# nihui/rife-ncnn-vulkan

Measured on AMD Instinct MI355X. Metric: interpolated frames/sec (rife-v4.6, 3840x2160), higher is better.
Workload: dtype f16x2-split MFMA + f32 accumulate (fp32-equivalent; activations stored f32 or as {hi, lo} f16 pairs); 1 GPU; rife-v4.6 3840x2160 frame pairs resident in HBM, timestep sweep [0.5, 0.125, 0.25, 0.7, 0.9], synthetic seeded weights; pairs_in_flight_per_gpu=4, cu_partition=every stream owns 1 / 2 of the compute units (rife_hip_stream_create), frames=F1: images/0.png, 1.png of the reference tiled 6 x 6, parallelism=frame pairs sharded over ranks, no data-path collective

## Files before the change

### rife-ncnn-vulkan_amd/__init__.py

```python
import ctypes
import os

import numpy as np

_HERE = os.path.dirname(os.path.abspath(__file__))
LIB_PATH = os.environ.get("RIFE_HIP_LIB") or os.path.join(_HERE, "librife_hip.so")
TEST_LIB_PATH = os.path.join(_HERE, "librife_hip_test.so")
_lib = None
_testlib = None

C_ABI_SYMBOLS = [
    "rife_hip_device_count", "rife_hip_create", "rife_hip_destroy", "rife_hip_load", "rife_hip_process",
    "rife_hip_process_device", "rife_hip_process_device_batch", "rife_hip_stream_create", "rife_hip_stream_destroy", "rife_hip_process_batch", "rife_hip_frame_upload", "rife_hip_process_frames", "rife_hip_frame_release",
    "rife_hip_last_error", "rife_hip_profile_enable", "rife_hip_profile_read",
    "rife_hip_host_alloc", "rife_hip_host_free", "rife_hip_host_register", "rife_hip_host_unregister",
    "rife_hip_graph_check", "rife_hip_param_hash",
    "rife_hip_frame_bytes", "rife_hip_process_px", "rife_hip_process_device_px", "rife_hip_process_device_batch_px", "rife_hip_frame_upload_px",
    "rife_hip_image_check", "rife_hip_image_row_bytes", "rife_hip_process_image", "rife_hip_process_device_image", "rife_hip_frame_upload_image", "rife_hip_process_frames_image",
]
PIX_RGB8, PIX_RGB10_U16, PIX_A2B10G10R10 = 0, 1, 2
PIX_RGBA8 = 4
PIX_NV12, PIX_I420, PIX_P010, PIX_I420P10 = 16, 17, 18, 19
PIX_I422, PIX_I422P10, PIX_I444, PIX_I444P10 = 33, 35, 49, 51
_YUV_FORMATS = (PIX_NV12, PIX_I420, PIX_P010, PIX_I420P10, PIX_I422, PIX_I422P10, PIX_I444, PIX_I444P10)
# ... 526 lines not shown
        _check(self._L.rife_hip_profile_enable(self._h, int(on)), "profile_enable", self._L)

    def profile_read(self):
        names = ctypes.create_string_buffer(4096)
        ms = np.zeros(64, np.float64); n = np.zeros(64, np.int64); fl = np.zeros(64, np.float64)
        k = self._L.rife_hip_profile_read(self._h, names, 4096, _p(ms), _p(n), _p(fl), 64)
        nm = names.value.decode().split("\n")
        return {nm[i]: dict(ms=float(ms[i]), launches=int(n[i]), flops=float(fl[i])) for i in range(k)}

    def _need_taps(self):
        if not self._taps:
            raise RifeError("the parity taps (include/rife_hip_test.h) live in the test build: create the engine with amd.test_build().RIFE(...)")

    def pool_state(self):
        self._need_taps()
        a, b, c = ctypes.c_int(), ctypes.c_int(), ctypes.c_int()
        _check(self._L.rife_hip_pool_state(self._h, ctypes.byref(a), ctypes.byref(b), ctypes.byref(c)), "pool_state", self._L)
        return a.value, b.value, c.value

    def v4_extract_flow(self, in0image, in1image, timestep, fi, inject=(), pixfmt=None):
        self._need_taps()
        px = _pix_of(in0image, pixfmt)
        if px is not None and _pix_of(in1image, px) != px:
            raise ValueError("both frames must have the same pixel format")
        if px is not None:
            a = np.ascontiguousarray(in0image); b = np.ascontiguousarray(in1image)
        else:
            a = np.ascontiguousarray(in0image, dtype=np.uint8); b = np.ascontiguousarray(in1image, dtype=np.uint8)
        h, w = a.shape[:2]
        nc, fh, fw = ctypes.c_int(), ctypes.c_int(), ctypes.c_int()
        _check(self._L.rife_hip_v4_flow_dims(self._h, w, h, fi, ctypes.byref(nc), ctypes.byref(fh), ctypes.byref(fw)), "v4_flow_dims", self._L)
        out = np.empty((nc.value, fh.value, fw.value), np.float32)
        inj = [np.ascontiguousarray(f, dtype=np.float32) for f in inject]
        arr = (ctypes.c_void_p * max(1, len(inj)))(*[f.ctypes.data for f in inj])
        if px is not None:
            _check(self._L.rife_hip_v4_extract_flow_px(self._h, _p(a), _p(b), w, h, float(timestep), fi, arr, len(inj), _p(out), px), "v4_extract_flow_px", self._L)
            return out
        _check(self._L.rife_hip_v4_extract_flow(self._h, _p(a), _p(b), w, h, float(timestep), fi, arr, len(inj), _p(out)), "v4_extract_flow", self._L)
        return out


    def v4_tap(self, in0image, in1image, timestep, what, b, inject, pixfmt=None):
        self._need_taps()
        px = _pix_of(in0image, pixfmt)
        if px is not None and _pix_of(in1image, px) != px:
            raise ValueError("both frames must have the same pixel format")
        if px is not None:
            a = np.ascontiguousarray(in0image); bb = np.ascontiguousarray(in1image)
        else:
            a = np.ascontiguousarray(in0image, dtype=np.uint8); bb = np.ascontiguousarray(in1image, dtype=np.uint8)
        h, w = a.shape[:2]
        wp, hp = (w + 31) // 32 * 32, (h + 31) // 32 * 32
        s = {1: 4, 2: 2, 3: 1}.get(b, 1)
        out = np.empty((4 if px == PIX_RGBA8 else 3, hp, wp) if what == 2 else (5, hp, wp) if what in (3, 4) else (12, hp // s, wp // s), np.float32)
        inj = [np.ascontiguousarray(f, dtype=np.float32) for f in inject]
        arr = (ctypes.c_void_p * max(1, len(inj)))(*[f.ctypes.data for f in inj])
        if px is not None:
            _check(self._L.rife_hip_v4_tap_px(self._h, _p(a), _p(bb), w, h, float(timestep), int(what), int(b), arr, len(inj), _p(out), px), "v4_tap_px", self._L)
            return out
        _check(self._L.rife_hip_v4_tap(self._h, _p(a), _p(bb), w, h, float(timestep), int(what), int(b), arr, len(inj), _p(out)), "v4_tap", self._L)
        return out

    def v4_process_injected(self, in0image, in1image, timestep, inject):
        self._need_taps()
        a = np.ascontiguousarray(in0image, dtype=np.uint8); bb = np.ascontiguousarray(in1image, dtype=np.uint8)
        h, w, _ = a.shape
        out = np.empty((h, w, 3), np.uint8)
        inj = [np.ascontiguousarray(f, dtype=np.float32) for f in inject]
        arr = (ctypes.c_void_p * max(1, len(inj)))(*[f.ctypes.data for f in inj])
        _check(self._L.rife_hip_v4_process_injected(self._h, _p(a), _p(bb), w, h, float(timestep), arr, len(inj), _p(out)), "v4_process_injected", self._L)
        return out


def op_conv3x3(x, weight, bias, stride=1, residual=None, slope=None, gpuid=0):
    x = np.ascontiguousarray(x, np.float32); weight = np.ascontiguousarray(weight, np.float32); bias = np.ascontiguousarray(bias, np.float32)
    c, h, w = x.shape
    oc = weight.shape[0]
    out = np.empty((oc, (h - 1) // stride + 1, (w - 1) // stride + 1), np.float32)
    res = None if residual is None else np.ascontiguousarray(residual, np.float32)
    sl = None if slope is None else np.ascontiguousarray(slope, np.float32)
    _check(testlib().rife_hip_op_conv3x3(gpuid, _p(x), c, h, w, _p(weight), _p(bias), oc, stride, _p(res), _p(sl), _p(out)), "op_conv3x3", testlib())
    return out


def op_deconv4x4(x, weight, bias, slope=None, gpuid=0):
    x = np.ascontiguousarray(x, np.float32); weight = np.ascontiguousarray(weight, np.float32); bias = np.ascontiguousarray(bias, np.float32)
    c, h, w = x.shape
    oc = weight.shape[0]
    out = np.empty((oc, 2 * h, 2 * w), np.float32)
    sl = None if slope is None else np.ascontiguousarray(slope, np.float32)
    _check(testlib().rife_hip_op_deconv4x4(gpuid, _p(x), c, h, w, _p(weight), _p(bias), oc, _p(sl), _p(out)), "op_deconv4x4", testlib())
    return out


def op_warp(image, flow, gpuid=0):
    image = np.ascontiguousarray(image, np.float32); flow = np.ascontiguousarray(flow, np.float32)
    c, h, w = image.shape
    out = np.empty_like(image)
    _check(testlib().rife_hip_op_warp(gpuid, _p(image), _p(flow), c, h, w, _p(out)), "op_warp", testlib())
    return out


def op_s16_geom(C, H, W):
    pitch, rows, plane, nbytes = ctypes.c_int(), ctypes.c_int(), ctypes.c_uint(), ctypes.c_size_t()
    _check(testlib().rife_hip_op_s16_geom(int(C), int(H), int(W), ctypes.byref(pitch), ctypes.byref(rows), ctypes.byref(plane), ctypes.byref(nbytes)), "op_s16_geom", testlib())
    return pitch.value, rows.value, plane.value, nbytes.value

# ... 50 lines not shown
```

### rife-ncnn-vulkan_amd/csrc/elementwise.h

```cpp
#pragma once
#include <hip/hip_runtime.h>
#include <stdint.h>

namespace rife {

__global__ void k_preproc(const uint8_t* __restrict__ rgb, int w, int h, uint32_t* __restrict__ out, int wp, int hp) {
    const int x = blockIdx.x * blockDim.x + threadIdx.x, y = blockIdx.y;
    if (x >= wp) return;
    uint32_t v = 0;
    if (x < w && y < h) {
        const uint8_t* p = rgb + ((size_t)y * w + x) * 3;
        v = (uint32_t)p[0] | ((uint32_t)p[1] << 8) | ((uint32_t)p[2] << 16);
    }
    out[(size_t)y * wp + x] = v;
}

__global__ void k_preproc4(const uint8_t* __restrict__ rgb, int w, int h, uint32_t* __restrict__ out, int wp, int hp) {
    const int x4 = (blockIdx.x * blockDim.x + threadIdx.x) * 4, y = blockIdx.y;
    if (x4 >= wp) return;
    uint4 v = make_uint4(0u, 0u, 0u, 0u);
    if (x4 < w && y < h) {
        typedef uint32_t u32x3 __attribute__((ext_vector_type(3)));
        u32x3 q;
        __builtin_memcpy(&q, __builtin_assume_aligned(rgb + ((size_t)y * w + x4) * 3, 4), 12);
// ... 150 lines not shown
    const int x = blockIdx.x * blockDim.x + threadIdx.x, y = blockIdx.y;
    if (x >= w) return;
    const size_t plane = (size_t)w * h;
    const WarpTaps t = warp_taps(x, y, flow[(size_t)y * w + x], flow[plane + (size_t)y * w + x], w, h);
    for (int q = 0; q < c; q++) {
        const float* im = image + q * plane;
        out[q * plane + (size_t)y * w + x] = warp_lerp(im[t.i00], im[t.i01], im[t.i10], im[t.i11], t.alpha, t.beta);
    }
}

__device__ __forceinline__ float down4(float v00, float v01, float v10, float v11) {
    const float r0 = v00 * 0.5f + v01 * 0.5f;
    const float r1 = v10 * 0.5f + v11 * 0.5f;
    return r0 * 0.5f + r1 * 0.5f;
}

template <int D>
__device__ __forceinline__ void assemble0_body(const uint32_t* __restrict__ img0, const uint32_t* __restrict__ img1, float timestep_arg, const float* __restrict__ tsp,
                                               float* __restrict__ X, int wp, int hp) {
    const float timestep = tsp ? *tsp : timestep_arg;
    const int Wb = wp / 8, Hb = hp / 8;
    const int x = blockIdx.x * blockDim.x + threadIdx.x, y = blockIdx.y;
    if (x >= Wb || y >= Hb) return;
    const int sx = 8 * x + 3, sy = 8 * y + 3;
    const size_t i00 = (size_t)sy * wp + sx, i10 = i00 + wp;
    const float3 a0 = unpack_rgb<D>(img0[i00]), a1 = unpack_rgb<D>(img0[i00 + 1]), a2 = unpack_rgb<D>(img0[i10]), a3 = unpack_rgb<D>(img0[i10 + 1]);
    const float3 b0 = unpack_rgb<D>(img1[i00]), b1 = unpack_rgb<D>(img1[i00 + 1]), b2 = unpack_rgb<D>(img1[i10]), b3 = unpack_rgb<D>(img1[i10 + 1]);
    float4 o0, o1;
    o0.x = down4(a0.x, a1.x, a2.x, a3.x); o0.y = down4(a0.y, a1.y, a2.y, a3.y); o0.z = down4(a0.z, a1.z, a2.z, a3.z);
    o0.w = down4(b0.x, b1.x, b2.x, b3.x); o1.x = down4(b0.y, b1.y, b2.y, b3.y); o1.y = down4(b0.z, b1.z, b2.z, b3.z);
    o1.z = down4(timestep, timestep, timestep, timestep);
    o1.w = 0.f;
    float4* dst = reinterpret_cast<float4*>(X + ((size_t)y * Wb + x) * 8);
    dst[0] = o0; dst[1] = o1;
}
__global__ void k_assemble0(const uint32_t* __restrict__ img0, const uint32_t* __restrict__ img1, float timestep_arg, const float* __restrict__ tsp,
                            float* __restrict__ X, int wp, int hp) {
    assemble0_body<8>(img0, img1, timestep_arg, tsp, X, wp, hp);
}
__global__ void k_assemble0_d10(const uint32_t* __restrict__ img0, const uint32_t* __restrict__ img1, float timestep_arg, const float* __restrict__ tsp,
                                float* __restrict__ X, int wp, int hp) {
    assemble0_body<10>(img0, img1, timestep_arg, tsp, X, wp, hp);
}

__device__ __forceinline__ void up_coeff(int d, int S, int in, int& s0, float& a0, float& a1) {
    float f = ((float)d + 0.5f) * (1.0f / (float)S) - 0.5f;
    int s = (int)floorf(f);
    f -= (float)s;
    if (s < 0) { s = 0; f = 0.f; }
    if (s >= in - 1) { s = in - 2; f = 1.f; }
    s0 = s; a0 = 1.f - f; a1 = f;
}

template <int S>
__device__ __forceinline__ void flow_upsampled(const float* __restrict__ flow, int wp, int hp, int x, int y, float4& u, float& um) {
    const int Wb = wp / S, Hb = hp / S;
    int sx, sy; float a0, a1, b0, b1;
    up_coeff(x, S, Wb, sx, a0, a1);
    up_coeff(y, S, Hb, sy, b0, b1);
    const float* p00 = flow + ((size_t)sy * Wb + sx) * 8;
    const float* p10 = p00 + (size_t)Wb * 8;
    const float4 q00 = *reinterpret_cast<const float4*>(p00), q01 = *reinterpret_cast<const float4*>(p00 + 8);
    const float4 q10 = *reinterpret_cast<const float4*>(p10), q11 = *reinterpret_cast<const float4*>(p10 + 8);
    const float m00 = p00[4], m01 = p00[12], m10 = p10[4], m11 = p10[12];
#define RIFE_UP(c00, c01, c10, c11) (((c00) * a0 + (c01) * a1) * b0 + ((c10) * a0 + (c11) * a1) * b1)
    u.x = RIFE_UP(q00.x, q01.x, q10.x, q11.x);
    u.y = RIFE_UP(q00.y, q01.y, q10.y, q11.y);
    u.z = RIFE_UP(q00.z, q01.z, q10.z, q11.z);
    u.w = RIFE_UP(q00.w, q01.w, q10.w, q11.w);
    um = RIFE_UP(m00, m01, m10, m11);
#undef RIFE_UP
}
template <int S>
__device__ __forceinline__ void flow_first(const float* __restrict__ flow, int wp, int hp, int x, int y, float4& f, float& m) {
    float4 u; float um;
    flow_upsampled<S>(flow, wp, hp, x, y, u, um);
    const float s = (float)S;
    f = make_float4(u.x * s, u.y * s, u.z * s, u.w * s);
    m = um;
}
template <int S>
__device__ __forceinline__ void flow_accumulate(const float4 u, const float um, float4& f, float& m) {
    const float s = (float)S;
    f = make_float4(f.x * 1.0f + u.x * s, f.y * 1.0f + u.y * s, f.z * 1.0f + u.z * s, f.w * 1.0f + u.w * s);
    m = m + um;
}

struct FlowPending {
    const float* flow = nullptr;
    float4* Fw = nullptr;
    float* Mw = nullptr;
};

template <int S, int UPD = 0, int D = 8>
__device__ __forceinline__ void assemble_pixel(const uint32_t* __restrict__ img0, const uint32_t* __restrict__ img1, float timestep,
                                               const float4* __restrict__ F, const float* __restrict__ M, int wp, int hp, int x, int y, float o[12],
                                               const FlowPending& pend = FlowPending{}) {
    if (S == 1) {
        const size_t i = (size_t)y * wp + x;
        float4 f; float mk;
        if (UPD == 2) flow_first<2 * S>(pend.flow, wp, hp, x, y, f, mk);
        else { f = F[i]; mk = M[i]; }
        if (UPD == 1) {
            float4 u; float um;
            flow_upsampled<2 * S>(pend.flow, wp, hp, x, y, u, um);
            flow_accumulate<2 * S>(u, um, f, mk);
            pend.Fw[i] = f; pend.Mw[i] = mk;
        }
        const float3 w0 = warp_rgbx<D>(img0, x, y, f.x, f.y, wp, hp);
        const float3 w1 = warp_rgbx<D>(img1, x, y, f.z, f.w, wp, hp);
        o[0] = w0.x; o[1] = w0.y; o[2] = w0.z; o[3] = w1.x; o[4] = w1.y; o[5] = w1.z; o[6] = timestep; o[7] = mk;
        o[8] = f.x; o[9] = f.y; o[10] = f.z; o[11] = f.w;
    } else {
        const int sx = S * x + S / 2 - 1, sy = S * y + S / 2 - 1;
        float v[4][12];
#pragma unroll
        for (int k = 0; k < 4; k++) {
            const int px = sx + (k & 1), py = sy + (k >> 1);
            const size_t i = (size_t)py * wp + px;
            float4 f; float mk;
            if (UPD == 2) flow_first<2 * S>(pend.flow, wp, hp, px, py, f, mk);
            else { f = F[i]; mk = M[i]; }
            if (UPD == 1) {
                float4 u; float um;
                flow_upsampled<2 * S>(pend.flow, wp, hp, px, py, u, um);
                flow_accumulate<2 * S>(u, um, f, mk);
                pend.Fw[i] = f; pend.Mw[i] = mk;
            }
            const float3 w0 = warp_rgbx<D>(img0, px, py, f.x, f.y, wp, hp);
            const float3 w1 = warp_rgbx<D>(img1, px, py, f.z, f.w, wp, hp);
            v[k][0] = w0.x; v[k][1] = w0.y; v[k][2] = w0.z; v[k][3] = w1.x; v[k][4] = w1.y; v[k][5] = w1.z;
            v[k][6] = timestep; v[k][7] = mk;
// ... 344 lines not shown
```

### rife-ncnn-vulkan_amd/csrc/engine.hip

```cpp
#include <hip/hip_runtime.h>

#include <algorithm>
#include <chrono>
#include <climits>
#include <cmath>
#include <cstdio>
#include <cstring>
#include <initializer_list>
#include <array>
#include <map>
#include <memory>
#include <atomic>
#include <mutex>
#include <string>
#include <thread>
#include <vector>

#if defined(RIFE_HIP_BENCH_BUILD) && !defined(RIFE_HIP_TEST_BUILD)
#define RIFE_HIP_TEST_BUILD 1
#endif
#include "../../include/rife_hip.h"
#ifdef RIFE_HIP_TEST_BUILD
#include "../../include/rife_hip_test.h"
#endif
#include "conv_mfma.h"
#include "conv_img.h"
#include "elementwise.h"
#include "yuv.h"
#include "planes.h"
#include "image_check.h"
#include "elementwise_v2.h"
#include "stem_fused.h"
#include "stem_fused_v2.h"
#include "stem_rs.h"
#include "tail_rs.h"
#include "head_h2.h"
#include "conv_t64.h"
#include "conv_row.h"
#include "conv_rs.h"
#include "conv_rs2.h"
#ifdef RIFE_HIP_TEST_BUILD
#include "conv_ks.h"
#endif
#include "graph_kernels.h"
#include "model_hashes.h"
#include "ncnn_model.h"

#include "engine_switches.h"
#include "engine_layers.h"
#include "engine_dispatch.h"
#include "engine_ctx.h"
#include "engine_v4.h"
#include "engine_v2.h"
#include "engine_v1.h"
#include "engine_abi.h"
#include "engine_image.h"
```

### rife-ncnn-vulkan_amd/csrc/engine_abi.h

```cpp

extern "C" {

const char* rife_hip_last_error(void) { return g_err.c_str(); }

int rife_hip_device_count(void) {
    int n = 0;
    if (hipGetDeviceCount(&n) != hipSuccess) return 0;
    return n;
}

rife_hip_t* rife_hip_create(int gpuid, int tta_mode, int tta_temporal_mode, int uhd_mode, int num_threads, int rife_v2, int rife_v4) {
    if (check_device(gpuid)) return nullptr;
    rife_hip* E = new rife_hip;
    E->gpuid = gpuid; E->tta = tta_mode; E->tta_temporal = tta_temporal_mode; E->uhd = uhd_mode;
    E->num_threads = num_threads; E->v2 = rife_v2; E->v4 = rife_v4;
    E->frame_pool = std::make_shared<FramePool>();
    E->frame_pool->gpuid = gpuid;
    const Switches sw = read_switches();
    E->t64 = sw.t64; E->rs = sw.rs; E->rs2 = sw.rs2; E->stem_rs = sw.stem_rs; E->tta_consensus = sw.tta_consensus;
    E->tail_rs = sw.tail_rs; E->tail_rs_always = sw.tail_rs_always; E->fuse_flow = sw.fuse_flow;
    if (sw.ks_mask >= 0) E->ks_mask = sw.ks_mask;
    if (E->fuse_flow) g_fuse_flow_buffers = true;
    return E;
}
// ... 768 lines not shown
    return n;
}

#ifdef RIFE_HIP_TEST_BUILD
static int rife_hip_v4_extract_flow_impl(const rife_hip_t* E, const uint8_t* in0, const uint8_t* in1, int w, int h, float timestep, int fi,
                                         const float* const* inject, int n_inject, float* out6chw, int pixfmt) {
    int rc;
    if ((rc = process_common(E, w, h, timestep))) return rc;
    if (!E->v4) return fail(RIFE_HIP_EINVAL, "stage taps exist for the rife-v4 family only");
    if (pix_bpp(pixfmt) == 0) return fail(RIFE_HIP_EINVAL, "unknown pixel format");
    if ((rc = pixfmt_supported(E, pixfmt))) return rc;
    if (fi < 0 || fi > 3 || n_inject < 0 || n_inject > fi) return fail(RIFE_HIP_EINVAL, "bad stage index");
    if ((rc = check_device(E->gpuid))) return rc;
    Ctx c;
    if (hipStreamCreateWithFlags(&c.stream, hipStreamNonBlocking) != hipSuccess) return fail(RIFE_HIP_EHIP, "hipStreamCreate failed");
    c.own_stream = true;
    if ((rc = ensure_ctx(c, w, h, pixfmt))) return rc;
    const size_t nbytes = frame_bytes(w, h, pixfmt);
    HIPCHK(hipMemcpyAsync(c.d_in0, in0, nbytes, hipMemcpyHostToDevice, c.stream));
    HIPCHK(hipMemcpyAsync(c.d_in1, in1, nbytes, hipMemcpyHostToDevice, c.stream));
    launch_preproc(c.stream, c.d_in0, c.w, c.h, c.img0, c.wp, c.hp, pixfmt);
    launch_preproc(c.stream, c.d_in1, c.w, c.h, c.img1, c.wp, c.hp, pixfmt);
    float* tmp = nullptr;
    if ((rc = dalloc(c, tmp, (size_t)c.wp * c.hp * 6))) return rc;
    const int nc = E->v40 ? 5 : 6;
    for (int b = 0; b <= fi; b++) {
        const int s = E->flow_div(b), Hb = c.hp / s, Wb = c.wp / s;
        if (b < n_inject) {
            HIPCHK(hipMemcpyAsync(tmp, inject[b], (size_t)Hb * Wb * nc * 4, hipMemcpyHostToDevice, c.stream));
            hipLaunchKernelGGL(k_chw_to_nhwc, grid2d(Wb, Hb), dim3(256), 0, c.stream, tmp, c.flow[b], nc, Hb, Wb, 8);
        } else {
            if ((rc = run_block_convs(*E, c, b, timestep))) return rc;
        }
        if (b < fi && (rc = run_flow_update(*E, c, b))) return rc;
    }
    const int s = E->flow_div(fi), Hb = c.hp / s, Wb = c.wp / s;
    hipLaunchKernelGGL(k_nhwc_to_chw, grid2d(Wb, Hb), dim3(256), 0, c.stream, c.flow[fi], tmp, nc, Hb, Wb, 8);
    HIPCHK(hipMemcpyAsync(out6chw, tmp, (size_t)Hb * Wb * nc * 4, hipMemcpyDeviceToHost, c.stream));
    HIPCHK(hipStreamSynchronize(c.stream));
    return 0;
}
int rife_hip_v4_extract_flow(const rife_hip_t* E, const uint8_t* in0, const uint8_t* in1, int w, int h, float timestep, int fi,
                             const float* const* inject, int n_inject, float* out6chw) {
    return rife_hip_v4_extract_flow_impl(E, in0, in1, w, h, timestep, fi, inject, n_inject, out6chw, RIFE_HIP_PIX_RGB8);
}
int rife_hip_v4_extract_flow_px(const rife_hip_t* E, const void* in0, const void* in1, int w, int h, float timestep, int fi, const float* const* inject,
                                int n_inject, float* out6chw, int pixfmt) {
    if (!in0 || !in1 || !out6chw) return fail(RIFE_HIP_EINVAL, "null frame / output pointer");
    try { return rife_hip_v4_extract_flow_impl(E, static_cast<const uint8_t*>(in0), static_cast<const uint8_t*>(in1), w, h, timestep, fi, inject, n_inject, out6chw, pixfmt); }
    catch (const std::exception& e) { return fail(RIFE_HIP_EINVAL, std::string("v4_extract_flow_px: ") + e.what()); }
}

static int tap_prologue(const rife_hip_t* E, Ctx& c, const uint8_t* in0, const uint8_t* in1, int w, int h, const float* const* inject, int n_inject, float*& tmp,
                        const float** pending = nullptr, int pixfmt = RIFE_HIP_PIX_RGB8) {
    int rc;
    if (hipStreamCreateWithFlags(&c.stream, hipStreamNonBlocking) != hipSuccess) return fail(RIFE_HIP_EHIP, "hipStreamCreate failed");
    c.own_stream = true;
    if ((rc = ensure_ctx(c, w, h, pixfmt))) return rc;
    const size_t nbytes = frame_bytes(w, h, pixfmt);
    HIPCHK(hipMemcpyAsync(c.d_in0, in0, nbytes, hipMemcpyHostToDevice, c.stream));
    HIPCHK(hipMemcpyAsync(c.d_in1, in1, nbytes, hipMemcpyHostToDevice, c.stream));
    launch_preproc(c.stream, c.d_in0, c.w, c.h, c.img0, c.wp, c.hp, pixfmt);
    launch_preproc(c.stream, c.d_in1, c.w, c.h, c.img1, c.wp, c.hp, pixfmt);
    if ((rc = dalloc(c, tmp, (size_t)c.wp * c.hp * 16))) return rc;
    for (int k = 0; k < n_inject; k++) {
        const int s = E->blk[k].scale, Hb = c.hp / s, Wb = c.wp / s;
        HIPCHK(hipMemcpyAsync(tmp, inject[k], (size_t)Hb * Wb * 6 * 4, hipMemcpyHostToDevice, c.stream));
        hipLaunchKernelGGL(k_chw_to_nhwc, grid2d(Wb, Hb), dim3(256), 0, c.stream, tmp, c.flow[k], 6, Hb, Wb, 8);
        if (pending && k == n_inject - 1 && k < 3 && flow_update_fused_into(*E, c, k + 1)) { *pending = c.flow[k]; continue; }
        if (k < 3 && (rc = run_flow_update(*E, c, k))) return rc;
    }
    HIPCHK(hipGetLastError());
    return 0;
}

static int rife_hip_v4_tap_impl(const rife_hip_t* E, const uint8_t* in0, const uint8_t* in1, int w, int h, float timestep, int what, int b,
                                const float* const* inject, int n_inject, float* out, int pixfmt = RIFE_HIP_PIX_RGB8) {
    int rc;
    if ((rc = process_common(E, w, h, timestep))) return rc;
    if (!E->v4 || E->v40) return fail(RIFE_HIP_EINVAL, "the gather taps exist for the rife-v4.6 graph only");
    if (pix_bpp(pixfmt) == 0) return fail(RIFE_HIP_EINVAL, "unknown pixel format");
    if ((rc = pixfmt_supported(E, pixfmt))) return rc;
    if (pixfmt && what == 3) return fail(RIFE_HIP_EINVAL, "tap 3 (an A/B form the product does not run) is served for RGB8 frames only");
    if (what < 0 || what > 5) return fail(RIFE_HIP_EINVAL, "bad tap");
    if (what == 5 && b != 3) return fail(RIFE_HIP_EINVAL, "the row-streaming stem kernel serves block 3");
    if (what == 2 ? n_inject != 4 : (b < 1 || b > 3 || n_inject != b)) return fail(RIFE_HIP_EINVAL, "bad block / injection count");
    if ((rc = check_device(E->gpuid))) return rc;
    Ctx c; float* tmp = nullptr;
    const float* pending = nullptr;
    if ((rc = tap_prologue(E, c, in0, in1, w, h, inject, n_inject, tmp, (what == 1 || what == 3) ? &pending : nullptr, pixfmt))) return rc;
    hipStream_t st = c.stream;
    auto copy_fm = [&](const float4* F, const float* M) -> int {
        hipLaunchKernelGGL(k_nhwc_to_chw, grid2d(c.wp, c.hp), dim3(256), 0, st, reinterpret_cast<const float*>(F), tmp, 4, c.hp, c.wp, 4);
        HIPCHK(hipGetLastError());
        const size_t P = (size_t)c.wp * c.hp;
        HIPCHK(hipMemcpyAsync(out, tmp, P * 16, hipMemcpyDeviceToHost, st));
        HIPCHK(hipMemcpyAsync(out + 4 * P, M, P * 4, hipMemcpyDeviceToHost, st));
        HIPCHK(hipStreamSynchronize(st));
        return 0;
    };
    if (what == 4) return copy_fm(c.F, c.M);
    if (what == 5) {
        const int Hq = c.hp / 4, Wq = c.wp / 4;
        const S16Geom G(Hq, Wq);
        const size_t nb = G.bytes(64), pl = G.plane();
        unsigned char* dout = nullptr; uint16_t *dw0 = nullptr, *dw1 = nullptr; float *dbias = nullptr, *dslope = nullptr;
        if ((rc = dalloc(c, dout, nb)) || (rc = dalloc(c, dw0, (size_t)9 * 2 * 32 * 8)) || (rc = dalloc(c, dw1, (size_t)2 * 9 * 2 * 64 * 8)) ||
            (rc = dalloc(c, dbias, 64)) || (rc = dalloc(c, dslope, 64))) return rc;
        std::vector<float> hz(64, 0.f), ho(64, 1.f);
        HIPCHK(hipMemcpyAsync(dbias, hz.data(), 256, hipMemcpyHostToDevice, st));
        HIPCHK(hipMemcpyAsync(dslope, ho.data(), 256, hipMemcpyHostToDevice, st));
        HIPCHK(hipFuncSetAttribute(reinterpret_cast<const void*>(stem_rs_kernel<0>), hipFuncAttributeMaxDynamicSharedMemorySize, SRS_LDS));
        HIPCHK(hipFuncSetAttribute(reinterpret_cast<const void*>(stem_rs_kernel<0, 10>), hipFuncAttributeMaxDynamicSharedMemorySize, SRS_LDS));
        std::vector<unsigned char> host(nb);
        int inv[32];
        for (int i = 0; i < 32; i++) inv[s16_row_channel(i)] = i;
        for (int g = 0; g < 2; g++)
            for (int ty = 1; ty <= 2; ty++)
                for (int tx = 1; tx <= 2; tx++) {
                    std::vector<uint16_t> h0((size_t)9 * 2 * 32 * 8, 0), h1((size_t)2 * 9 * 2 * 64 * 8, 0);
                    for (int j = 0; j < 2; j++)
                        for (int k = 0; k < 12; k++) h0[(((size_t)((1 + g) * 3 + 1 + j) * 2 + k / 8) * 32 + 12 * j + k) * 8 + k % 8] = f2h(1.f);
                    for (int oc = 0; oc < 24; oc++)
                        h1[((((size_t)(oc / 16) * 9 + ty * 3 + tx) * 2 + (oc % 16) / 8) * 64 + inv[oc]) * 8 + oc % 8] = f2h(1.f);
                    HIPCHK(hipMemcpyAsync(dw0, h0.data(), h0.size() * 2, hipMemcpyHostToDevice, st));
                    HIPCHK(hipMemcpyAsync(dw1, h1.data(), h1.size() * 2, hipMemcpyHostToDevice, st));
                    HIPCHK(hipMemsetAsync(dout, 0, nb, st));
                    StemRsArgs a;
                    a.img0 = c.img0; a.img1 = c.img1; a.F = c.F; a.M = c.M; a.w0 = dw0; a.bias0 = dbias; a.slope0 = dslope; a.w1 = dw1; a.bias1 = dbias; a.slope1 = dslope;
                    a.out = dout; a.timestep = timestep; a.tsp = nullptr; a.wp = c.wp; a.hp = c.hp; a.Hq = Hq; a.Wq = Wq; a.pitch = G.pitch; a.plane = G.plane();
                    a.nunits = ((Wq + SRS_SW - 1) / SRS_SW) * Hq;
                    const int nwg = std::min(2 * device_cus(), a.nunits);
                    if (pix_deep(pixfmt)) hipLaunchKernelGGL((stem_rs_kernel<0, 10>), dim3(nwg), dim3(SRS_NTHR), SRS_LDS, st, a);
                    else hipLaunchKernelGGL((stem_rs_kernel<0>), dim3(nwg), dim3(SRS_NTHR), SRS_LDS, st, a);
                    HIPCHK(hipGetLastError());
                    HIPCHK(hipMemcpyAsync(host.data(), dout, nb, hipMemcpyDeviceToHost, st));
                    HIPCHK(hipStreamSynchronize(st));
                    for (int j = 0; j < 2; j++)
                        for (int k = 0; k < 12; k++) {
                            const int oc = 12 * j + k;
                            const _Float16* hi = reinterpret_cast<const _Float16*>(host.data() + (size_t)(2 * (oc / 16)) * pl);
                            const _Float16* lo = reinterpret_cast<const _Float16*>(host.data() + (size_t)(2 * (oc / 16) + 1) * pl);
                            for (int q = 0; q < Hq; q++)
                                for (int x = 0; x < Wq; x++) {
                                    const size_t e = ((size_t)(q + 1) * G.pitch + x + 1) * 16 + oc % 16;
                                    out[((size_t)k * c.hp + 4 * q + 2 * (ty - 1) + g) * c.wp + 4 * x + 2 * (tx - 1) + j] = (float)hi[e] + (float)lo[e];
                                }
                        }
                }
        return 0;
    }
    if (what == 3 && !pending) return fail(RIFE_HIP_EINVAL, "the flow update before this block is not fused into its stem");
    if (what == 2) {
        float4* outf = nullptr;
// ... 370 lines not shown
```

### rife-ncnn-vulkan_amd/csrc/engine_switches.h

```cpp

namespace rife {


static thread_local std::string g_err;
static int fail(int code, const std::string& msg) { g_err = msg; return -code; }

struct Switches {
    bool trunk_h2;
    bool use_graph;
    int batch_workers;
    bool v2_stem16;
    int ns3_rows4, rows4_max;
    bool t64_loader_waves;
    bool rs_split;
    int ks_div;
    bool ctx0_img;
    bool v2_ctx_batch;
    bool v2_fused_stem;
    bool v2_stem_r64;
    bool v2_skip_copy;
    int tta_lane_parts;
    bool h2d_token;
    int pool_parts;
    bool t64, rs, rs2, stem_rs, tta_consensus, tail_rs, tail_rs_always, fuse_flow;
    int ks_mask;
    bool merge_flow0;
    int batch_groups;
    bool profile_fine;
    int probe_lds; const char* probe_scrub; bool probe_quiet;
};
static Switches read_switches() {
    auto on = [](const char* e) { return e && e[0] == '1'; };
    auto not_off = [](const char* e) { return !(e && e[0] == '0'); };
    auto num = [](const char* e, int dflt, int lo, int hi) { if (!e) return dflt; const int v = atoi(e); return v >= lo && v <= hi ? v : dflt; };
    auto ab = [](const char* name) -> const char* {
#ifdef RIFE_HIP_TEST_BUILD
        return getenv(name);
#else
        (void)name; return nullptr;
#endif
    };
    Switches s;
    { const char* e = getenv("RIFE_HIP_TRUNK"); s.trunk_h2 = !(e && std::strcmp(e, "f32") == 0); }
    s.use_graph = on(getenv("RIFE_HIP_GRAPH"));
    s.batch_workers = num(getenv("RIFE_HIP_BATCH_WORKERS"), 0, 1, 16);
    s.profile_fine = on(getenv("RIFE_HIP_PROFILE_FINE"));
    s.v2_stem16 = not_off(ab("RIFE_HIP_V2_STEM16"));
    s.ns3_rows4 = num(ab("RIFE_HIP_NS3_ROWS4"), 0, INT_MIN, INT_MAX);
    s.rows4_max = num(ab("RIFE_HIP_ROWS4_MAX"), 400, INT_MIN, INT_MAX);
    s.t64_loader_waves = on(ab("RIFE_HIP_T64_LW"));
    s.rs_split = on(ab("RIFE_HIP_RS_SPLIT"));
    s.ks_div = num(ab("RIFE_HIP_KS_DIV"), 1, 1, 8);
    s.ctx0_img = not_off(ab("RIFE_HIP_CTX0_IMG"));
    s.v2_ctx_batch = not_off(ab("RIFE_HIP_V2_CTX_BATCH"));
    s.v2_fused_stem = not_off(ab("RIFE_HIP_V2_FUSED_STEM"));
    s.v2_stem_r64 = not_off(ab("RIFE_HIP_V2_STEM_R64"));
    s.v2_skip_copy = on(ab("RIFE_HIP_V2_SKIP_COPY"));
    s.pool_parts = num(ab("RIFE_HIP_POOL_PARTS"), -1, 0, 4);
    s.h2d_token = not_off(ab("RIFE_HIP_H2D_TOKEN"));
    s.tta_lane_parts = num(ab("RIFE_HIP_TTA_LANE_PARTS"), 0, 0, 4);
    s.t64 = not_off(ab("RIFE_HIP_T64"));
    s.rs = not_off(ab("RIFE_HIP_RS"));
    s.rs2 = not_off(ab("RIFE_HIP_RS2"));
    { const char* e = ab("RIFE_HIP_KS"); s.ks_mask = e && e[0] >= '0' && e[0] <= '9' ? atoi(e) : -1; }
    s.stem_rs = not_off(ab("RIFE_HIP_STEM_RS"));
    s.tta_consensus = not_off(ab("RIFE_HIP_TTA_CONSENSUS"));
    { const char* e = ab("RIFE_HIP_TAIL_RS"); s.tail_rs = not_off(e); s.tail_rs_always = e && e[0] == '2'; }
    s.fuse_flow = on(ab("RIFE_HIP_FUSE_FLOW"));
    s.merge_flow0 = not_off(ab("RIFE_HIP_MERGE_FLOW0"));
    { const char* e = ab("RIFE_HIP_BATCH_GROUPS"); s.batch_groups = e ? (e[0] != '0' ? 1 : 0) : -1; }
    { const char* e = ab("RIFE_HIP_PROBE_LDS"); s.probe_lds = e ? atoi(e) : -1; }
    s.probe_scrub = ab("RIFE_HIP_PROBE_SCRUB");
    s.probe_quiet = ab("RIFE_HIP_PROBE_QUIET") != nullptr;
    return s;
}
static const Switches& process_switches() { static const Switches s = read_switches(); return s; }

#define HIPCHK(x)                                                                                   \
    do {                                                                                            \
        hipError_t e_ = (x);                                                                        \
        if (e_ != hipSuccess) return fail(RIFE_HIP_EHIP, std::string(#x) + ": " + hipGetErrorString(e_)); \
    } while (0)

}
```

### rife-ncnn-vulkan_amd/csrc/engine_v4.h

```cpp

namespace rife {


static const uint64_t V46_HASH_OUT0 = RIFE_V46_HASH_OUT0;

static std::atomic<bool> g_fuse_flow_buffers{false};

static int ensure_ctx_dims_impl(Ctx& c, int w, int h, int wp, int hp, const Ctx* scratch, bool own_images, bool want_outf, size_t stage_bytes) {
    if (!c.v2 && c.wp == wp && c.hp == hp && c.w == w && c.h == h && (!want_outf || c.outf) && (scratch || c.stage_bytes >= stage_bytes)) return 0;
    c.stage_bytes = stage_bytes;
    c.v2 = false;
    if (c.gexec) { (void)hipGraphExecDestroy(c.gexec); c.gexec = nullptr; }
    c.g_warm = false; c.d_ts = nullptr;
    for (void* p : c.allocs) (void)hipFree(p);
    c.allocs.clear();
    c.outf = nullptr; c.F2 = nullptr; c.M2 = nullptr; c.yuv_rgb = nullptr;
    for (auto& pb : c.P) pb[0] = pb[1] = nullptr;
    c.w = w; c.h = h; c.wp = wp; c.hp = hp;
    const size_t P = (size_t)wp * hp;
    int rc;
    if (own_images) {
        if ((rc = dalloc(c, c.img0, P))) return rc;
        if ((rc = dalloc(c, c.img1, P))) return rc;
    }
// ... 336 lines not shown
    if (E.v40) {
        Timed t(E.prof, "v40_block_add", 0, st);
        const size_t n4 = (size_t)Ht * Wt * B.c / 4;
        hipLaunchKernelGGL(k_add_inplace, dim3((unsigned)((n4 + 255) / 256)), dim3(256), 0, st, reinterpret_cast<float4*>(cur), reinterpret_cast<const float4*>(c.T2), n4);
        HIPCHK(hipGetLastError());
    }
    {
        Timed t(E.prof, B.head.cls, B.head.flops_per_pixel * Ht * Wt, st);
        if ((rc = launch_conv(B.head, {cur, B.c, 0}, Ht, Wt, {c.flow[b], 8, 0}, nullptr, st, fin))) return rc;
    }
    return 0;
}

static int run_flow_update(const rife_hip& E, Ctx& c, int b) {
    hipStream_t st = c.stream;
    Timed t(E.prof, "flow_update", 0, st);
    dim3 g = grid2d(c.wp, c.hp);
    if (E.v40) {
        if (b == 0) hipLaunchKernelGGL((k_flow_update<16, true>), g, dim3(256), 0, st, c.flow[0], c.F, c.M, c.wp, c.hp);
        else if (b == 1) hipLaunchKernelGGL((k_flow_update<8, false>), g, dim3(256), 0, st, c.flow[1], c.F, c.M, c.wp, c.hp);
        else if (b == 2) hipLaunchKernelGGL((k_flow_update<4, false>), g, dim3(256), 0, st, c.flow[2], c.F, c.M, c.wp, c.hp);
        else hipLaunchKernelGGL((k_flow_update<2, false>), g, dim3(256), 0, st, c.flow[3], c.F, c.M, c.wp, c.hp);
        HIPCHK(hipGetLastError());
        return 0;
    }
    if (b == 0) hipLaunchKernelGGL((k_flow_update<8, true>), g, dim3(256), 0, st, c.flow[0], c.F, c.M, c.wp, c.hp);
    else if (b == 1) hipLaunchKernelGGL((k_flow_update<4, false>), g, dim3(256), 0, st, c.flow[1], c.F, c.M, c.wp, c.hp);
    else hipLaunchKernelGGL((k_flow_update<2, false>), g, dim3(256), 0, st, c.flow[2], c.F, c.M, c.wp, c.hp);
    HIPCHK(hipGetLastError());
    return 0;
}

static int run_v4(const rife_hip& E, Ctx& c, const uint8_t* d_in0, const uint8_t* d_in1, float timestep, uint8_t* d_out, const float* tsp = nullptr, const PlaneIO* pio = nullptr) {
    hipStream_t st = c.stream;
    int rc;
    {
        Timed t(E.prof, "preproc", 0, st);
        if (pio) {
            launch_preproc_planes(st, pio->in0, c.w, c.h, c.img0, c.wp, c.hp, c.pixfmt);
            launch_preproc_planes(st, pio->in1, c.w, c.h, c.img1, c.wp, c.hp, c.pixfmt);
        } else {
            launch_preproc(st, d_in0, c.w, c.h, c.img0, c.wp, c.hp, c.pixfmt);
            launch_preproc(st, d_in1, c.w, c.h, c.img1, c.wp, c.hp, c.pixfmt);
        }
        HIPCHK(hipGetLastError());
    }
    if (c.pixfmt && E.v40) return fail(RIFE_HIP_ENOSYS, "10-bit and RGBA frames are served for model family rife-v4.6 only, not rife-v4");
    const bool fuse_tail = !E.v40 && trunk_h2() && g_head_h2 && g_fuse_tail && E.blk[3].head.d_wh != nullptr;
    uint8_t* const caller_out = d_out;
    const int opf = pix_inner(c.pixfmt);
    if (pix_yuv(c.pixfmt)) d_out = reinterpret_cast<uint8_t*>(c.yuv_rgb);
    FinalArgs fin{c.img0, c.img1, c.F, c.M, d_out, c.w, c.h, c.wp, c.hp, opf};
    const float* pending = nullptr;
    const bool merge_env = read_switches().merge_flow0;
    const bool merge0 = merge_env && !E.v40 && trunk_h2() && g_fuse_stem && E.blk[1].stem0.d_wh != nullptr && E.blk[1].scale == 4 && !flow_update_fused_into(E, c, 1) &&
                        !flow_update_fused_into(E, c, 2);
    for (int b = 0; b < 4; b++) {
        if ((rc = run_block_convs(E, c, b, timestep, (b == 3 && fuse_tail) ? &fin : nullptr, tsp, PH_ALL, pending, (merge0 && b == 1) ? c.flow[0] : nullptr))) return rc;
        pending = nullptr;
        if (merge0 && b == 0) continue;
        if (merge0 && b == 1) {
            Timed t(E.prof, "flow_update", 0, st);
            hipLaunchKernelGGL((k_flow_update2<8, 4>), grid2d(c.wp, c.hp), dim3(256), 0, st, c.flow[0], c.flow[1], c.F, c.M, c.wp, c.hp);
            HIPCHK(hipGetLastError());
            continue;
        }
        if (b < 3 && flow_update_fused_into(E, c, b + 1)) pending = c.flow[b];
        else if ((b < 3 || E.v40) && (rc = run_flow_update(E, c, b))) return rc;
    }
    if (E.v40) {
        Timed t(E.prof, "final", 0, st);
        hipLaunchKernelGGL(k_blend_final, grid2d(c.w, c.h), dim3(256), 0, st, c.img0, c.img1, c.F, c.M, d_out, c.w, c.h, c.wp, c.hp);
        HIPCHK(hipGetLastError());
    } else if (!fuse_tail) {
        Timed t(E.prof, "final", 0, st);
        if (opf == RIFE_HIP_PIX_RGB10_U16) hipLaunchKernelGGL(k_final_px<1>, grid2d(c.w, c.h), dim3(256), 0, st, c.img0, c.img1, c.F, c.M, c.flow[3], d_out, c.w, c.h, c.wp, c.hp);
        else if (opf == RIFE_HIP_PIX_A2B10G10R10) hipLaunchKernelGGL(k_final_px<2>, grid2d(c.w, c.h), dim3(256), 0, st, c.img0, c.img1, c.F, c.M, c.flow[3], d_out, c.w, c.h, c.wp, c.hp);
        else if (opf == RIFE_HIP_PIX_RGBA8) hipLaunchKernelGGL(k_final_px<4>, grid2d(c.w, c.h), dim3(256), 0, st, c.img0, c.img1, c.F, c.M, c.flow[3], d_out, c.w, c.h, c.wp, c.hp);
        else hipLaunchKernelGGL(k_final, grid2d(c.w, c.h), dim3(256), 0, st, c.img0, c.img1, c.F, c.M, c.flow[3], d_out, c.w, c.h, c.wp, c.hp);
        HIPCHK(hipGetLastError());
    }
    if (pix_yuv(c.pixfmt)) {
        Timed t(E.prof, "postproc_yuv", 0, st);
        if (pio) launch_postproc_yuv_planes(st, c.yuv_rgb, c.w, c.h, pio->out, c.pixfmt);
        else launch_postproc_yuv(st, c.yuv_rgb, c.w, c.h, caller_out, c.pixfmt);
        HIPCHK(hipGetLastError());
    }
    return 0;
}

static int run_v4_group(const rife_hip& E, Ctx* const* cs, int G, const uint8_t* const* d_in0, const uint8_t* const* d_in1, const float* ts, uint8_t* const* d_out) {
    int rc;
    for (int g = 0; g < G; g++) {
        Ctx& c = *cs[g];
        if (!c.ev_group) HIPCHK(hipEventCreateWithFlags(&c.ev_group, hipEventDisableTiming));
        Timed t(E.prof, "preproc", 0, c.stream);
        launch_preproc(c.stream, d_in0[g], c.w, c.h, c.img0, c.wp, c.hp, c.pixfmt);
        launch_preproc(c.stream, d_in1[g], c.w, c.h, c.img1, c.wp, c.hp, c.pixfmt);
        HIPCHK(hipGetLastError());
    }
    const bool fuse_tail = trunk_h2() && g_head_h2 && g_fuse_tail && E.blk[3].head.d_wh != nullptr;
    const float* pend[4] = {nullptr, nullptr, nullptr, nullptr};
    auto after_block = [&](Ctx& c, int g, int b) -> int {
        if (b < 3 && flow_update_fused_into(E, c, b + 1)) { pend[g] = c.flow[b]; return 0; }
        return b < 3 ? run_flow_update(E, c, b) : 0;
    };
    for (int b = 0; b < 4; b++) {
        const rife_hip::Block& B = E.blk[b];
        const bool batched = G >= 2 && block_on_row_kernel(E, *cs[0], b) && block_on_s16(E, *cs[0], b);
        for (int g = 0; g < G; g++) {
            Ctx& c = *cs[g];
            FinalArgs fin{c.img0, c.img1, c.F, c.M, pix_yuv(c.pixfmt) ? reinterpret_cast<uint8_t*>(c.yuv_rgb) : d_out[g], c.w, c.h, c.wp, c.hp, pix_inner(c.pixfmt)};
            if (!batched) {
                if ((rc = run_block_convs(E, c, b, ts[g], (b == 3 && fuse_tail) ? &fin : nullptr, nullptr, PH_ALL, pend[g]))) return rc;
                pend[g] = nullptr;
                if ((rc = after_block(c, g, b))) return rc;
// ... 218 lines not shown
```

Before: 495.8 frames/s.

## Add LDS-staged flow cascade kernel recomputing F/M from low-res flows

Adds a tiled kernel that stages the coarse per-block flow cells for a 64x16 output tile into shared memory, then rebuilds the full-resolution accumulated flow F and mask M from scratch by upsampling and summing flows 0..2. After block 2 this replaces the incremental flow update, which had to read the full-resolution F/M back before adding the new level. The cascade is on by default, and block 1's merged update also moves to the tiled LDS kernel. The cost is extra per-pixel arithmetic for every level and LDS staging with a barrier, traded against one full-resolution read of F and M.

New measurement: 509.1 frames/s (median of 6 runs). +2.7%, better.

```diff
diff --git a/rife-ncnn-vulkan_amd/__init__.py b/rife-ncnn-vulkan_amd/__init__.py
--- a/rife-ncnn-vulkan_amd/__init__.py
+++ b/rife-ncnn-vulkan_amd/__init__.py
@@ -602,7 +602,7 @@
         h, w = a.shape[:2]
         wp, hp = (w + 31) // 32 * 32, (h + 31) // 32 * 32
         s = {1: 4, 2: 2, 3: 1}.get(b, 1)
-        out = np.empty((4 if px == PIX_RGBA8 else 3, hp, wp) if what == 2 else (5, hp, wp) if what in (3, 4) else (12, hp // s, wp // s), np.float32)
+        out = np.empty((4 if px == PIX_RGBA8 else 3, hp, wp) if what == 2 else (5, hp, wp) if what in (3, 4, 6) else (12, hp // s, wp // s), np.float32)
         inj = [np.ascontiguousarray(f, dtype=np.float32) for f in inject]
         arr = (ctypes.c_void_p * max(1, len(inj)))(*[f.ctypes.data for f in inj])
         if px is not None:
diff --git a/rife-ncnn-vulkan_amd/csrc/elementwise.h b/rife-ncnn-vulkan_amd/csrc/elementwise.h
--- a/rife-ncnn-vulkan_amd/csrc/elementwise.h
+++ b/rife-ncnn-vulkan_amd/csrc/elementwise.h
@@ -226,6 +226,7 @@
     s0 = s; a0 = 1.f - f; a1 = f;
 }
 
+#define RIFE_UP(c00, c01, c10, c11) (((c00) * a0 + (c01) * a1) * b0 + ((c10) * a0 + (c11) * a1) * b1)
 template <int S>
 __device__ __forceinline__ void flow_upsampled(const float* __restrict__ flow, int wp, int hp, int x, int y, float4& u, float& um) {
     const int Wb = wp / S, Hb = hp / S;
@@ -237,21 +238,34 @@
     const float4 q00 = *reinterpret_cast<const float4*>(p00), q01 = *reinterpret_cast<const float4*>(p00 + 8);
     const float4 q10 = *reinterpret_cast<const float4*>(p10), q11 = *reinterpret_cast<const float4*>(p10 + 8);
     const float m00 = p00[4], m01 = p00[12], m10 = p10[4], m11 = p10[12];
-#define RIFE_UP(c00, c01, c10, c11) (((c00) * a0 + (c01) * a1) * b0 + ((c10) * a0 + (c11) * a1) * b1)
     u.x = RIFE_UP(q00.x, q01.x, q10.x, q11.x);
     u.y = RIFE_UP(q00.y, q01.y, q10.y, q11.y);
     u.z = RIFE_UP(q00.z, q01.z, q10.z, q11.z);
     u.w = RIFE_UP(q00.w, q01.w, q10.w, q11.w);
     um = RIFE_UP(m00, m01, m10, m11);
+}
+__device__ __forceinline__ void flow_upsampled_cells(const float* p00, const float* p10, float a0, float a1, float b0, float b1, float4& u, float& um) {
+    const float4 q00 = *reinterpret_cast<const float4*>(p00), q01 = *reinterpret_cast<const float4*>(p00 + 8);
+    const float4 q10 = *reinterpret_cast<const float4*>(p10), q11 = *reinterpret_cast<const float4*>(p10 + 8);
+    const float m00 = p00[4], m01 = p00[12], m10 = p10[4], m11 = p10[12];
+    u.x = RIFE_UP(q00.x, q01.x, q10.x, q11.x);
+    u.y = RIFE_UP(q00.y, q01.y, q10.y, q11.y);
+    u.z = RIFE_UP(q00.z, q01.z, q10.z, q11.z);
+    u.w = RIFE_UP(q00.w, q01.w, q10.w, q11.w);
+    um = RIFE_UP(m00, m01, m10, m11);
+}
 #undef RIFE_UP
+template <int S>
+__device__ __forceinline__ void flow_first_of(const float4 u, const float um, float4& f, float& m) {
+    const float s = (float)S;
+    f = make_float4(u.x * s, u.y * s, u.z * s, u.w * s);
+    m = um;
 }
 template <int S>
 __device__ __forceinline__ void flow_first(const float* __restrict__ flow, int wp, int hp, int x, int y, float4& f, float& m) {
     float4 u; float um;
     flow_upsampled<S>(flow, wp, hp, x, y, u, um);
-    const float s = (float)S;
-    f = make_float4(u.x * s, u.y * s, u.z * s, u.w * s);
-    m = um;
+    flow_first_of<S>(u, um, f, m);
 }
 template <int S>
 __device__ __forceinline__ void flow_accumulate(const float4 u, const float um, float4& f, float& m) {
diff --git a/rife-ncnn-vulkan_amd/csrc/engine.hip b/rife-ncnn-vulkan_amd/csrc/engine.hip
--- a/rife-ncnn-vulkan_amd/csrc/engine.hip
+++ b/rife-ncnn-vulkan_amd/csrc/engine.hip
@@ -26,6 +26,7 @@
 #include "conv_mfma.h"
 #include "conv_img.h"
 #include "elementwise.h"
+#include "flow_cascade.h"
 #include "yuv.h"
 #include "planes.h"
 #include "image_check.h"
diff --git a/rife-ncnn-vulkan_amd/csrc/engine_abi.h b/rife-ncnn-vulkan_amd/csrc/engine_abi.h
--- a/rife-ncnn-vulkan_amd/csrc/engine_abi.h
+++ b/rife-ncnn-vulkan_amd/csrc/engine_abi.h
@@ -844,7 +844,7 @@
 }
 
 static int tap_prologue(const rife_hip_t* E, Ctx& c, const uint8_t* in0, const uint8_t* in1, int w, int h, const float* const* inject, int n_inject, float*& tmp,
-                        const float** pending = nullptr, int pixfmt = RIFE_HIP_PIX_RGB8) {
+                        const float** pending = nullptr, int pixfmt = RIFE_HIP_PIX_RGB8, bool updates = true) {
     int rc;
     if (hipStreamCreateWithFlags(&c.stream, hipStreamNonBlocking) != hipSuccess) return fail(RIFE_HIP_EHIP, "hipStreamCreate failed");
     c.own_stream = true;
@@ -859,6 +859,7 @@
         const int s = E->blk[k].scale, Hb = c.hp / s, Wb = c.wp / s;
         HIPCHK(hipMemcpyAsync(tmp, inject[k], (size_t)Hb * Wb * 6 * 4, hipMemcpyHostToDevice, c.stream));
         hipLaunchKernelGGL(k_chw_to_nhwc, grid2d(Wb, Hb), dim3(256), 0, c.stream, tmp, c.flow[k], 6, Hb, Wb, 8);
+        if (!updates) continue;
         if (pending && k == n_inject - 1 && k < 3 && flow_update_fused_into(*E, c, k + 1)) { *pending = c.flow[k]; continue; }
         if (k < 3 && (rc = run_flow_update(*E, c, k))) return rc;
     }
@@ -874,13 +875,14 @@
     if (pix_bpp(pixfmt) == 0) return fail(RIFE_HIP_EINVAL, "unknown pixel format");
     if ((rc = pixfmt_supported(E, pixfmt))) return rc;
     if (pixfmt && what == 3) return fail(RIFE_HIP_EINVAL, "tap 3 (an A/B form the product does not run) is served for RGB8 frames only");
-    if (what < 0 || what > 5) return fail(RIFE_HIP_EINVAL, "bad tap");
+    if (what < 0 || what > 6) return fail(RIFE_HIP_EINVAL, "bad tap");
+    if (what == 6 && b != 2 && b != 3) return fail(RIFE_HIP_EINVAL, "the flow cascade runs after block 1 (b = 2) or block 2 (b = 3)");
     if (what == 5 && b != 3) return fail(RIFE_HIP_EINVAL, "the row-streaming stem kernel serves block 3");
     if (what == 2 ? n_inject != 4 : (b < 1 || b > 3 || n_inject != b)) return fail(RIFE_HIP_EINVAL, "bad block / injection count");
     if ((rc = check_device(E->gpuid))) return rc;
     Ctx c; float* tmp = nullptr;
     const float* pending = nullptr;
-    if ((rc = tap_prologue(E, c, in0, in1, w, h, inject, n_inject, tmp, (what == 1 || what == 3) ? &pending : nullptr, pixfmt))) return rc;
+    if ((rc = tap_prologue(E, c, in0, in1, w, h, inject, n_inject, tmp, (what == 1 || what == 3) ? &pending : nullptr, pixfmt, what != 6))) return rc;
     hipStream_t st = c.stream;
     auto copy_fm = [&](const float4* F, const float* M) -> int {
         hipLaunchKernelGGL(k_nhwc_to_chw, grid2d(c.wp, c.hp), dim3(256), 0, st, reinterpret_cast<const float*>(F), tmp, 4, c.hp, c.wp, 4);
@@ -892,6 +894,12 @@
         return 0;
     };
     if (what == 4) return copy_fm(c.F, c.M);
+    if (what == 6) {
+        if (b == 2) launch_flow_cascade<2>(st, c.flow[0], c.flow[1], nullptr, c.F, c.M, c.wp, c.hp);
+        else launch_flow_cascade<3>(st, c.flow[0], c.flow[1], c.flow[2], c.F, c.M, c.wp, c.hp);
+        HIPCHK(hipGetLastError());
+        return copy_fm(c.F, c.M);
+    }
     if (what == 5) {
         const int Hq = c.hp / 4, Wq = c.wp / 4;
         const S16Geom G(Hq, Wq);
diff --git a/rife-ncnn-vulkan_amd/csrc/engine_switches.h b/rife-ncnn-vulkan_amd/csrc/engine_switches.h
--- a/rife-ncnn-vulkan_amd/csrc/engine_switches.h
+++ b/rife-ncnn-vulkan_amd/csrc/engine_switches.h
@@ -25,6 +25,7 @@
     bool t64, rs, rs2, stem_rs, tta_consensus, tail_rs, tail_rs_always, fuse_flow;
     int ks_mask;
     bool merge_flow0;
+    bool flow_cascade;
     int batch_groups;
     bool profile_fine;
     int probe_lds; const char* probe_scrub; bool probe_quiet;
@@ -68,6 +69,7 @@
     { const char* e = ab("RIFE_HIP_TAIL_RS"); s.tail_rs = not_off(e); s.tail_rs_always = e && e[0] == '2'; }
     s.fuse_flow = on(ab("RIFE_HIP_FUSE_FLOW"));
     s.merge_flow0 = not_off(ab("RIFE_HIP_MERGE_FLOW0"));
+    s.flow_cascade = not_off(ab("RIFE_HIP_FLOW_CASCADE"));
     { const char* e = ab("RIFE_HIP_BATCH_GROUPS"); s.batch_groups = e ? (e[0] != '0' ? 1 : 0) : -1; }
     { const char* e = ab("RIFE_HIP_PROBE_LDS"); s.probe_lds = e ? atoi(e) : -1; }
     s.probe_scrub = ab("RIFE_HIP_PROBE_SCRUB");
diff --git a/rife-ncnn-vulkan_amd/csrc/engine_v4.h b/rife-ncnn-vulkan_amd/csrc/engine_v4.h
--- a/rife-ncnn-vulkan_amd/csrc/engine_v4.h
+++ b/rife-ncnn-vulkan_amd/csrc/engine_v4.h
@@ -412,16 +412,25 @@
     if (pix_yuv(c.pixfmt)) d_out = reinterpret_cast<uint8_t*>(c.yuv_rgb);
     FinalArgs fin{c.img0, c.img1, c.F, c.M, d_out, c.w, c.h, c.wp, c.hp, opf};
     const float* pending = nullptr;
-    const bool merge_env = read_switches().merge_flow0;
+    const Switches sw = read_switches();
+    const bool merge_env = sw.merge_flow0;
     const bool merge0 = merge_env && !E.v40 && trunk_h2() && g_fuse_stem && E.blk[1].stem0.d_wh != nullptr && E.blk[1].scale == 4 && !flow_update_fused_into(E, c, 1) &&
                         !flow_update_fused_into(E, c, 2);
+    const bool cascade = merge0 && sw.flow_cascade && !flow_update_fused_into(E, c, 3);
     for (int b = 0; b < 4; b++) {
         if ((rc = run_block_convs(E, c, b, timestep, (b == 3 && fuse_tail) ? &fin : nullptr, tsp, PH_ALL, pending, (merge0 && b == 1) ? c.flow[0] : nullptr))) return rc;
         pending = nullptr;
         if (merge0 && b == 0) continue;
         if (merge0 && b == 1) {
             Timed t(E.prof, "flow_update", 0, st);
-            hipLaunchKernelGGL((k_flow_update2<8, 4>), grid2d(c.wp, c.hp), dim3(256), 0, st, c.flow[0], c.flow[1], c.F, c.M, c.wp, c.hp);
+            if (cascade) launch_flow_cascade<2>(st, c.flow[0], c.flow[1], nullptr, c.F, c.M, c.wp, c.hp);
+            else hipLaunchKernelGGL((k_flow_update2<8, 4>), grid2d(c.wp, c.hp), dim3(256), 0, st, c.flow[0], c.flow[1], c.F, c.M, c.wp, c.hp);
+            HIPCHK(hipGetLastError());
+            continue;
+        }
+        if (cascade && b == 2) {
+            Timed t(E.prof, "flow_update", 0, st);
+            launch_flow_cascade<3>(st, c.flow[0], c.flow[1], c.flow[2], c.F, c.M, c.wp, c.hp);
             HIPCHK(hipGetLastError());
             continue;
         }
diff --git a/rife-ncnn-vulkan_amd/csrc/flow_cascade.h b/rife-ncnn-vulkan_amd/csrc/flow_cascade.h
--- /dev/null
+++ b/rife-ncnn-vulkan_amd/csrc/flow_cascade.h
@@ -0,0 +1,73 @@
+#pragma once
+#include <hip/hip_runtime.h>
+
+#include "elementwise.h"
+#include "flow_cascade_geom.h"
+
+namespace rife {
+
+template <int L>
+__device__ __forceinline__ void cascade_stage(const float* __restrict__ flow, float4* cells, int x0, int y0, int wp, int hp, fcg::Span& sx, fcg::Span& sy) {
+    constexpr int S = fcg::scale(L), P2 = fcg::pitch(L) * 2, N2 = fcg::records(L) * 2;
+    const int Wb = wp / S;
+    sx = fcg::span(x0, fcg::TILE_W, wp, S);
+    sy = fcg::span(y0, fcg::TILE_H, hp, S);
+    const float4* src = reinterpret_cast<const float4*>(flow) + ((size_t)sy.lo * Wb + sx.lo) * 2;
+    float4* dst = cells + fcg::offset(L) * 2;
+    for (int j = threadIdx.x; j < N2; j += fcg::THREADS) {
+        const int r = j / P2, q = j - r * P2;
+        if (r < sy.n && q < 2 * sx.n) dst[j] = src[(size_t)r * Wb * 2 + q];
+    }
+}
+
+template <int L>
+__device__ __forceinline__ void cascade_sample(const float4* cells, const fcg::Span& sx, const fcg::Span& sy, int wp, int hp, int x, int y, float4& u, float& um) {
+    constexpr int S = fcg::scale(L);
+    int cx, cy; float a0, a1, b0, b1;
+    up_coeff(x, S, wp / S, cx, a0, a1);
+    up_coeff(y, S, hp / S, cy, b0, b1);
+    const float* p00 = reinterpret_cast<const float*>(cells + (fcg::offset(L) + (cy - sy.lo) * fcg::pitch(L) + (cx - sx.lo)) * 2);
+    flow_upsampled_cells(p00, p00 + fcg::pitch(L) * 8, a0, a1, b0, b1, u, um);
+}
+
+template <int NL>
+__global__ __launch_bounds__(fcg::THREADS) void k_flow_cascade(const float* __restrict__ flow0, const float* __restrict__ flow1, const float* __restrict__ flow2,
+                                                               float4* __restrict__ F, float* __restrict__ M, int wp, int hp) {
+    static_assert(NL == 2 || NL == 3, "the cascade after block 1 or after block 2");
+    __shared__ float4 cells[fcg::lds_records(NL) * 2];
+    const int x0 = blockIdx.x * fcg::TILE_W, y0 = blockIdx.y * fcg::TILE_H;
+    fcg::Span sx0, sy0, sx1, sy1, sx2 = {0, 0}, sy2 = {0, 0};
+    cascade_stage<0>(flow0, cells, x0, y0, wp, hp, sx0, sy0);
+    cascade_stage<1>(flow1, cells, x0, y0, wp, hp, sx1, sy1);
+    if (NL == 3) cascade_stage<2>(flow2, cells, x0, y0, wp, hp, sx2, sy2);
+    __syncthreads();
+    const int x = x0 + (threadIdx.x & 63);
+    if (x >= wp) return;
+    constexpr int ROWS = fcg::TILE_H / (fcg::THREADS / 64);
+    const int yw = y0 + (threadIdx.x >> 6) * ROWS;
+#pragma unroll
+    for (int k = 0; k < ROWS; k++) {
+        const int y = yw + k;
+        if (y >= hp) break;
+        float4 f, u; float m, um;
+        cascade_sample<0>(cells, sx0, sy0, wp, hp, x, y, u, um);
+        flow_first_of<8>(u, um, f, m);
+        cascade_sample<1>(cells, sx1, sy1, wp, hp, x, y, u, um);
+        flow_accumulate<4>(u, um, f, m);
+        if (NL == 3) {
+            cascade_sample<2>(cells, sx2, sy2, wp, hp, x, y, u, um);
+            flow_accumulate<2>(u, um, f, m);
+        }
+        const size_t i = (size_t)y * wp + x;
+        F[i] = f;
+        M[i] = m;
+    }
+}
+
+template <int NL>
+static inline void launch_flow_cascade(hipStream_t st, const float* flow0, const float* flow1, const float* flow2, float4* F, float* M, int wp, int hp) {
+    const dim3 g(fcg::tiles(wp, fcg::TILE_W), fcg::tiles(hp, fcg::TILE_H));
+    hipLaunchKernelGGL((k_flow_cascade<NL>), g, dim3(fcg::THREADS), 0, st, flow0, flow1, flow2, F, M, wp, hp);
+}
+
+}
diff --git a/rife-ncnn-vulkan_amd/csrc/flow_cascade_geom.h b/rife-ncnn-vulkan_amd/csrc/flow_cascade_geom.h
--- /dev/null
+++ b/rife-ncnn-vulkan_amd/csrc/flow_cascade_geom.h
@@ -0,0 +1,42 @@
+#pragma once
+
+#if defined(__HIPCC__)
+#define FCG_HD __host__ __device__
+#else
+#define FCG_HD
+#endif
+
+namespace fcg {
+
+constexpr int TILE_W = 64;
+constexpr int TILE_H = 16;
+constexpr int THREADS = 256;
+constexpr int LEVELS = 3;
+
+FCG_HD constexpr int scale(int l) { return 8 >> l; }
+FCG_HD constexpr int pitch(int l) { return TILE_W / scale(l) + 2; }
+FCG_HD constexpr int rows(int l) { return TILE_H / scale(l) + 2; }
+FCG_HD constexpr int records(int l) { return pitch(l) * rows(l); }
+FCG_HD constexpr int offset(int l) { return l == 0 ? 0 : offset(l - 1) + records(l - 1); }
+FCG_HD constexpr int lds_records(int levels) { return offset(levels); }
+
+FCG_HD inline int up_s0(int d, int S, int in) {
+    const int num = 2 * d + 1 - S;
+    int s = num < 0 ? 0 : num / (2 * S);
+    if (s >= in - 1) s = in - 2;
+    return s;
+}
+
+struct Span { int lo, n; };
+FCG_HD inline Span span(int d0, int tile, int full, int S) {
+    const int in = full / S;
+    const int d1 = (d0 + tile < full ? d0 + tile : full) - 1;
+    Span r;
+    r.lo = up_s0(d0, S, in);
+    r.n = up_s0(d1, S, in) + 2 - r.lo;
+    return r;
+}
+
+FCG_HD inline int tiles(int full, int tile) { return (full + tile - 1) / tile; }
+
+}
```
